# nv-tlabs/LION

Hardware: AMD Instinct MI355X
Metric: shapes/sec @1000-step DDIM, Bx2048pts (higher is better)
Workload: dtype f32 (operands of the 3x3x3 voxel convolutions and of the long 1x1 convolutions cut into fp16 hi/lo pairs on the 16-bi...

## Files before the change

include/lion_hip.h:

```cpp
#ifndef LION_HIP_H_
#define LION_HIP_H_

#include <stddef.h>
#include <stdint.h>

#ifdef __cplusplus
extern "C" {
#endif

typedef void *lionStream_t;

#define LION_OK 0
#define LION_EINVAL (-1)
#define LION_EUNSUPPORTED (-2)
#define LION_EWORKSPACE (-3)

int lion_abi_version(void);

size_t lion_avg_voxelize_workspace_bytes(int B, int C, int N, int r);
int lion_avg_voxelize_forward(const float *feat, const int32_t *coords, int B, int C, int N,
                              int r, float *out, int32_t *ind, int32_t *cnt, void *ws,
                              size_t ws_bytes, lionStream_t stream);

int lion_voxelize_points_forward(const float *feat, const float *coords, int B, int C, int N,
// ... 167 lines not shown
int lion_groupnorm_fold(const float *stats, int B, int C, int T, int G, int voxels, const float *gamma,
                        const float *beta, const float *fac, const float *gbias, int ld_fg, float eps,
                        float *A, float *Bs, float *chmean, lionStream_t stream);
size_t lion_conv3d_split_packed_halfs(int Cout, int Cin);
int lion_conv3d_split_pack_weights(const float *w, int Cout, int Cin, uint16_t *wp, lionStream_t stream);
int lion_conv3d_split_stat_tiles(int r, int Cout);
int lion_conv3d_k3_split_forward(const float *x, const uint16_t *wp, const float *bias, int B, int Cin, int Cout,
                                 int r, const float *pro_a, const float *pro_b, const float *pro_bias,
                                 const float *tconst, float *y, float *stats, int32_t *occ, lionStream_t stream);
int lion_conv3d_k3_half_forward(const float *x, const uint16_t *wp, const float *bias, int B, int Cin, int Cout,
                                int r, const float *pro_a, const float *pro_b, const float *pro_bias,
                                const float *tconst, float *y, float *stats, int32_t *occ, lionStream_t stream);
size_t lion_skinny_packed_floats(int Cout, int Cin);
int lion_skinny_pack_weights(const float *w, int Cout, int Cin, float *wp, lionStream_t stream);
int lion_skinny_splits(int Cin, int Cout);
int lion_skinny_gemm(const float *pin, int ks_in, const float *bias_in, int act_in, const float *addT,
                     const float *wp, int nb, int Cin, int Cout, float *pout, lionStream_t stream);
int lion_skinny_finish(const float *A, int ks_a, const float *bias_a, const float *Bp, int ks_b, const float *resid,
                       int nb, int C, int mode, float *y, lionStream_t stream);
int lion_skinny_gemm_se_finish(const float *pin, int ks_in, const float *bias_in, int act_in, const float *wp, int nb, int Cin,
                               int Cout, const float *A, int ks_a, const float *bias_a, const float *resid, float *y,
                               lionStream_t stream);
int lion_internal_skinny_gemm_plain(const float *pin, int ks_in, const float *bias_in, int act_in, const float *addT,
                                    const float *wp, int nb, int Cin, int Cout, float *pout, lionStream_t stream);
int lion_internal_skinny_gemm_se_finish_plain(const float *pin, int ks_in, const float *bias_in, int act_in, const float *wp,
                                              int nb, int Cin, int Cout, const float *A, int ks_a, const float *bias_a,
                                              const float *resid, float *y, lionStream_t stream);
int lion_to_channel_major(const float *a, int lda, int Ca, float *oa, const float *b, int ldb, int Cb, float *ob, int B,
                          lionStream_t stream);
int lion_from_channel_major(const float *x, int B, int C, float *y, lionStream_t stream);
int lion_groupnorm_fold_se(const float *stats, int B, int C, int T, int G, int voxels, const float *gamma,
                           const float *beta, const float *fac, const float *gbias, int ld_fg, float eps, const float *w1,
                           const float *w2, int H, float *A, float *Bs, lionStream_t stream);
int lion_se_gate(const float *chmean, const float *w1, const float *w2, int B, int C, int H, float *A,
                 float *Bs, lionStream_t stream);
int lion_trilinear_devoxelize_affine_forward(const float *coords, const float *feat, const float *scale,
                                             const float *shift, int B, int C, int N, int r, float *out,
                                             lionStream_t stream);
size_t lion_devoxelize_plan_bytes(int B, int N, int r);
int lion_trilinear_devoxelize_plan(const float *coords, int B, int N, int r, void *plan, size_t plan_bytes,
                                   lionStream_t stream);
int lion_trilinear_devoxelize_planned_forward(const void *plan, size_t plan_bytes, const float *coords, const float *feat,
                                              const float *scale, const float *shift, int B, int C, int N, int r,
                                              float *out, lionStream_t stream);

int lion_row_stats(const float *x, int rows, int L, float *stats, lionStream_t stream);
size_t lion_pwconv_packed_floats(int Cout, int Cin);
int lion_pwconv_pack_weights(const float *w, int Cout, int Cin, float *wp, lionStream_t stream);
int lion_pwconv_stat_tiles(int Cout, int Cin, int L);
int lion_pwconv_forward(const float *x, const float *wp, const float *bias, int B, int Cin, int Cout, int L,
                        const float *pro_a, const float *pro_b, float *y, float *stats, lionStream_t stream);
int lion_pwconv_forward_max(const float *x, const float *wp, const float *bias, int B, int Cin, int Cout, int L,
                            const float *pro_a, const float *pro_b, const float *out_a, const float *out_b,
                            float *stats, float *ymax, lionStream_t stream);
size_t lion_pwconv_split_packed_halfs(int Cout, int Cin);
int lion_pwconv_split_pack_weights(const float *w, int Cout, int Cin, uint16_t *wp, lionStream_t stream);
int lion_pwconv_split_pack_weights_t(const float *w, int Cout, int Cin, const uint16_t *wp, uint16_t *wpt, lionStream_t stream);
int lion_pwconv_split_stat_tiles(int Cout, int Cin, int L);
int lion_pwconv_split_forward(const float *x, const uint16_t *wp, const float *bias, int B, int Cin, int Cout, int L,
                              const float *pro_a, const float *pro_b, float *y, float *stats, lionStream_t stream);
int lion_pwconv_grouped_forward(const float *coords, const float *centers, const float *feat, const int32_t *idx,
                                const float *wp, const float *bias, int B, int C, int N, int M, int U, int Cout, float *y,
                                float *stats, lionStream_t stream);
int lion_pwconv_split_grouped_forward(const float *coords, const float *centers, const float *feat, const int32_t *idx,
                                      const uint16_t *wp, const float *bias, int B, int C, int N, int M, int U, int Cout,
                                      float *y, float *stats, lionStream_t stream);
int lion_internal_pwconv_walk(const float *x, const float *wp, const float *bias, int B, int Cin, int Cout, int L,
                              const float *pro_a, const float *pro_b, const float *out_a, const float *out_b,
                              const float *coords, const float *centers, const float *feat, const int32_t *idx, int N, int U,
                              float *y, float *stats, int max_wg, int lds_weights, lionStream_t stream);
int lion_linear_attention_core(const float *qkv, int B, int H, int D, int N, float *out, lionStream_t stream);
int lion_internal_linear_attention_path(int N, int aligned);
int lion_internal_linear_attention_core_plain(const float *qkv, int B, int H, int D, int N, float *out, lionStream_t stream);
int lion_linear_attention_core_backward(const float *qkv, const float *gout, int B, int H, int D, int N, float *gqkv,
                                        lionStream_t stream);
int lion_linear_forward(const float *x, const float *wp, const float *bias, int B, int K, int O, int act, float slope,
                        float *y, lionStream_t stream);
int lion_affine_swish(const float *x, const float *A, const float *Bs, int rows, int L, float *y,
                      lionStream_t stream);
int lion_affine_swish_max(const float *x, const float *A, const float *Bs, int rows, int M, int U,
                          float *y, lionStream_t stream);
int lion_timestep_embedding(const float *t, const float *row, float scale, int B, int half, int D, float *emb,
                            lionStream_t stream);
int lion_affine_swish_add(const float *x, const float *A, const float *Bs, const float *addend, int rows, int L, float *y,
                          lionStream_t stream);

size_t lion_scatter_csr_workspace_bytes(int B, int E, int bins);
int lion_scatter_csr(const float *gy, const int32_t *idx, const float *w, int B, int C, int S, int E, int bins, void *ws,
                     size_t ws_bytes, float *gx, lionStream_t stream);

size_t lion_pwconv_wgrad_workspace_bytes(int B, int Cin, int Cout, int L);
int lion_pwconv_wgrad(const float *x, const float *gy, int B, int Cin, int Cout, int L, void *ws, size_t ws_bytes,
                      float *gw, float *gb, lionStream_t stream);

int lion_gn_train_fold(const float *stats, const float *gw, const float *gb, const float *fac, int fac_stride,
                       const float *bias, int bias_stride, int B, int C, int G, int L, float eps, float *A, float *Bs,
                       float *mean, float *rstd, lionStream_t stream);
int lion_row_stats64(const float *x, int rows, int L, double *stats, lionStream_t stream);
int lion_gn_train_fold64(const double *stats, const float *gw, const float *gb, const float *fac, int fac_stride,
                         const float *bias, int bias_stride, int B, int C, int G, int L, float eps, float *A,
                         float *Bs, float *mean, float *rstd, lionStream_t stream);
int lion_gn_train_bwd_fold(const float *S, const float *mean, const float *rstd, const float *gw, const float *gb,
                           const float *fac, int fac_stride, int B, int C, int G, int L, float *Q, float *R, float *dfac,
// ... 74 lines not shown
```

lion_amd/_lib.py:

```python
from __future__ import annotations

import ctypes as C
import os

_HERE = os.path.dirname(os.path.abspath(__file__))
SO_PATH = os.environ.get("LION_HIP_SO") or os.path.join(_HERE, "csrc", "liblion_hip.so")

_vp, _i, _f, _sz = C.c_void_p, C.c_int, C.c_float, C.c_size_t

SIGNATURES = {
    "lion_abi_version": (_i, []),
    "lion_avg_voxelize_workspace_bytes": (_sz, [_i, _i, _i, _i]),
    "lion_avg_voxelize_forward": (_i, [_vp, _vp, _i, _i, _i, _i, _vp, _vp, _vp, _vp, _sz, _vp]),
    "lion_voxelize_points_forward": (_i, [_vp, _vp, _i, _i, _i, _i, _i, _f, _vp, _vp, _vp, _vp,
                                          _vp, _sz, _vp]),
    "lion_voxel_plan_bytes": (_sz, [_i, _i, _i]),
    "lion_voxel_index": (_i, [_vp, _i, _i, _i, _i, _f, _vp, _vp, _vp, _vp, _sz, _vp]),
    "lion_voxel_scatter": (_i, [_vp, _vp, _sz, _i, _i, _i, _i, _vp, _vp]),
    "lion_voxel_scatter_read": (_i, [_vp, _vp, _sz, _i, _i, _i, _i, _vp, _vp, _vp]),
    "lion_avg_voxelize_backward": (_i, [_vp, _vp, _vp, _i, _i, _i, _i, _vp, _vp]),
    "lion_trilinear_devoxelize_forward": (_i, [_vp, _vp, _i, _i, _i, _i, _i, _vp, _vp, _vp, _vp]),
    "lion_trilinear_devoxelize_backward": (_i, [_vp, _vp, _vp, _i, _i, _i, _i, _vp, _vp]),
    "lion_ball_query": (_i, [_vp, _vp, _i, _i, _i, _f, _i, _vp, _vp]),
    "lion_grouping_forward": (_i, [_vp, _vp, _i, _i, _i, _i, _i, _vp, _vp]),
# ... 4 lines not shown
    "lion_gather_features_backward": (_i, [_vp, _vp, _i, _i, _i, _i, _vp, _vp]),
    "lion_three_nn_interpolate_forward": (_i, [_vp, _vp, _vp, _i, _i, _i, _i, _vp, _vp, _vp, _vp]),
    "lion_three_nn_interpolate_backward": (_i, [_vp, _vp, _vp, _i, _i, _i, _i, _vp, _vp]),
    "lion_chamfer_forward": (_i, [_vp, _vp, _i, _i, _i, _vp, _vp, _vp, _vp, _vp]),
    "lion_chamfer_backward": (_i, [_vp, _vp, _vp, _vp, _vp, _vp, _i, _i, _i, _vp, _vp, _vp]),
    "lion_chamfer_loss_reduce": (_i, [_vp, _vp, _i, _i, _i, _f, _f, _vp, _vp]),
    "lion_chamfer_loss_backward": (_i, [_vp, _vp, _vp, _vp, _vp, _i, _i, _i, _f, _f, _vp, _vp, _vp]),
    "lion_emd_workspace_bytes": (_sz, [_i, _i, _i]),
    "lion_emd_approxmatch": (_i, [_vp, _vp, _i, _i, _i, _vp, _vp, _sz, _vp]),
    "lion_emd_cost": (_i, [_vp, _vp, _i, _i, _i, _vp, _vp, _sz, _vp]),
    "lion_emd_matchcost": (_i, [_vp, _vp, _vp, _i, _i, _i, _vp, _vp, _sz, _vp]),
    "lion_emd_matchcost_backward": (_i, [_vp, _vp, _vp, _vp, _i, _i, _i, _vp, _vp, _vp]),
    "lion_conv3d_packed_floats": (_sz, [_i, _i]),
    "lion_conv3d_pack_weights": (_i, [_vp, _i, _i, _vp, _vp]),
    "lion_conv3d_k3_forward": (_i, [_vp, _vp, _vp, _i, _i, _i, _i, _vp, _vp]),
    "lion_conv3d_wgrad_workspace_floats": (_sz, [_i, _i, _i, _i]),
    "lion_conv3d_k3_wgrad": (_i, [_vp, _vp, _i, _i, _i, _i, _vp, _vp, _sz, _vp]),
    "lion_conv3d_k3_wgrad_split": (_i, [_vp, _vp, _i, _i, _i, _i, _vp, _vp, _sz, _vp]),
    "lion_conv3d_wgrad_sparse_workspace_floats": (_sz, [_i, _i, _i, _i]),
    "lion_conv3d_k3_wgrad_split_sparse": (_i, [_vp, _vp, _vp, _i, _i, _i, _i, _vp, _vp, _sz, _vp]),
    "lion_conv3d_stat_tiles": (_i, [_i, _i, _i, _i]),
    "lion_conv3d_k3_fused_forward": (_i, [_vp, _vp, _vp, _i, _i, _i, _i, _vp, _vp, _vp, _vp, _vp, _vp, _vp, _vp]),
    "lion_conv3d_const_response": (_i, [_vp, _vp, _vp, _vp, _vp, _i, _i, _i, _vp, _vp]),
    "lion_conv3d_occupancy_ints": (_sz, [_i, _i, _i]),
    "lion_conv3d_tile_occupancy": (_i, [_vp, _i, _i, _i, _vp, _vp, _vp]),
    "lion_conv3d_tile_occupancy_aware": (_i, [_vp, _i, _i, _i, _vp, _vp, _i, _vp]),
    "lion_conv3d_split_packed_halfs": (_sz, [_i, _i]),
    "lion_conv3d_split_pack_weights": (_i, [_vp, _i, _i, _vp, _vp]),
    "lion_conv3d_split_stat_tiles": (_i, [_i, _i]),
    "lion_conv3d_k3_split_forward": (_i, [_vp, _vp, _vp, _i, _i, _i, _i, _vp, _vp, _vp, _vp, _vp, _vp, _vp, _vp]),
    "lion_conv3d_k3_half_forward": (_i, [_vp, _vp, _vp, _i, _i, _i, _i, _vp, _vp, _vp, _vp, _vp, _vp, _vp, _vp]),
    "lion_groupnorm_fold": (_i, [_vp, _i, _i, _i, _i, _i, _vp, _vp, _vp, _vp, _i, _f, _vp, _vp, _vp, _vp]),
    "lion_groupnorm_fold_se": (_i, [_vp, _i, _i, _i, _i, _i, _vp, _vp, _vp, _vp, _i, _f, _vp, _vp, _i, _vp, _vp, _vp]),
    "lion_skinny_packed_floats": (_sz, [_i, _i]),
    "lion_skinny_pack_weights": (_i, [_vp, _i, _i, _vp, _vp]),
    "lion_skinny_splits": (_i, [_i, _i]),
    "lion_skinny_gemm": (_i, [_vp, _i, _vp, _i, _vp, _vp, _i, _i, _i, _vp, _vp]),
    "lion_skinny_gemm_se_finish": (_i, [_vp, _i, _vp, _i, _vp, _i, _i, _i, _vp, _i, _vp, _vp, _vp, _vp]),
    "lion_internal_skinny_gemm_plain": (_i, [_vp, _i, _vp, _i, _vp, _vp, _i, _i, _i, _vp, _vp]),
    "lion_internal_skinny_gemm_se_finish_plain": (_i, [_vp, _i, _vp, _i, _vp, _i, _i, _i, _vp, _i, _vp, _vp, _vp, _vp]),
    "lion_skinny_finish": (_i, [_vp, _i, _vp, _vp, _i, _vp, _i, _i, _i, _vp, _vp]),
    "lion_to_channel_major": (_i, [_vp, _i, _i, _vp, _vp, _i, _i, _vp, _i, _vp]),
    "lion_from_channel_major": (_i, [_vp, _i, _i, _vp, _vp]),
    "lion_se_gate": (_i, [_vp, _vp, _vp, _i, _i, _i, _vp, _vp, _vp]),
    "lion_trilinear_devoxelize_affine_forward": (_i, [_vp, _vp, _vp, _vp, _i, _i, _i, _i, _vp, _vp]),
    "lion_devoxelize_plan_bytes": (_sz, [_i, _i, _i]),
    "lion_trilinear_devoxelize_plan": (_i, [_vp, _i, _i, _i, _vp, _sz, _vp]),
    "lion_trilinear_devoxelize_planned_forward": (_i, [_vp, _sz, _vp, _vp, _vp, _vp, _i, _i, _i, _i, _vp, _vp]),
    "lion_row_stats": (_i, [_vp, _i, _i, _vp, _vp]),
    "lion_pwconv_packed_floats": (_sz, [_i, _i]),
    "lion_pwconv_pack_weights": (_i, [_vp, _i, _i, _vp, _vp]),
    "lion_pwconv_stat_tiles": (_i, [_i, _i, _i]),
    "lion_pwconv_forward": (_i, [_vp, _vp, _vp, _i, _i, _i, _i, _vp, _vp, _vp, _vp, _vp]),
    "lion_pwconv_forward_max": (_i, [_vp, _vp, _vp, _i, _i, _i, _i, _vp, _vp, _vp, _vp, _vp, _vp, _vp]),
    "lion_pwconv_split_packed_halfs": (_sz, [_i, _i]),
    "lion_pwconv_split_pack_weights": (_i, [_vp, _i, _i, _vp, _vp]),
    "lion_pwconv_split_pack_weights_t": (_i, [_vp, _i, _i, _vp, _vp, _vp]),
    "lion_pwconv_split_stat_tiles": (_i, [_i, _i, _i]),
    "lion_pwconv_split_forward": (_i, [_vp, _vp, _vp, _i, _i, _i, _i, _vp, _vp, _vp, _vp, _vp]),
    "lion_pwconv_grouped_forward": (_i, [_vp, _vp, _vp, _vp, _vp, _vp, _i, _i, _i, _i, _i, _i, _vp, _vp, _vp]),
    "lion_pwconv_split_grouped_forward": (_i, [_vp, _vp, _vp, _vp, _vp, _vp, _i, _i, _i, _i, _i, _i, _vp, _vp, _vp]),
    "lion_internal_pwconv_walk": (_i, [_vp, _vp, _vp, _i, _i, _i, _i, _vp, _vp, _vp, _vp, _vp, _vp, _vp, _vp, _i, _i, _vp, _vp, _i, _i, _vp]),
    "lion_linear_attention_core": (_i, [_vp, _i, _i, _i, _i, _vp, _vp]),
    "lion_internal_linear_attention_path": (_i, [_i, _i]),
    "lion_internal_linear_attention_core_plain": (_i, [_vp, _i, _i, _i, _i, _vp, _vp]),
    "lion_linear_attention_core_backward": (_i, [_vp, _vp, _i, _i, _i, _i, _vp, _vp]),
    "lion_linear_forward": (_i, [_vp, _vp, _vp, _i, _i, _i, _i, _f, _vp, _vp]),
    "lion_affine_swish": (_i, [_vp, _vp, _vp, _i, _i, _vp, _vp]),
    "lion_affine_swish_max": (_i, [_vp, _vp, _vp, _i, _i, _i, _vp, _vp]),
    "lion_timestep_embedding": (_i, [_vp, _vp, _f, _i, _i, _i, _vp, _vp]),
    "lion_affine_swish_add": (_i, [_vp, _vp, _vp, _vp, _i, _i, _vp, _vp]),
    "lion_scatter_csr_workspace_bytes": (_sz, [_i, _i, _i]),
    "lion_scatter_csr": (_i, [_vp, _vp, _vp, _i, _i, _i, _i, _i, _vp, _sz, _vp, _vp]),
    "lion_pwconv_wgrad_workspace_bytes": (_sz, [_i, _i, _i, _i]),
    "lion_pwconv_wgrad": (_i, [_vp, _vp, _i, _i, _i, _i, _vp, _sz, _vp, _vp, _vp]),
    "lion_gn_train_fold": (_i, [_vp, _vp, _vp, _vp, _i, _vp, _i, _i, _i, _i, _i, _f, _vp, _vp, _vp, _vp, _vp]),
    "lion_row_stats64": (_i, [_vp, _i, _i, _vp, _vp]),
    "lion_gn_train_fold64": (_i, [_vp, _vp, _vp, _vp, _i, _vp, _i, _i, _i, _i, _i, _f, _vp, _vp, _vp, _vp, _vp]),
    "lion_gn_train_bwd_fold": (_i, [_vp, _vp, _vp, _vp, _vp, _vp, _i, _i, _i, _i, _i, _vp, _vp, _vp, _vp, _i, _vp, _vp, _vp, _vp, _vp,
                                    _vp, _vp]),
    "lion_gn_train_param_grads": (_i, [_vp, _i, _i, _vp, _vp, _vp, _vp]),
    "lion_adam_chunk": (_i, []),
    "lion_adam_row": (_i, []),
    "lion_adam_step": (_i, [_vp, _vp, _vp, _i, _i, _vp, _f, _f, _f, _f, _f, _vp]),
    "lion_grad_sqnorm_partials": (_i, [_vp, _vp, _vp, _i, _vp, _vp]),
    "lion_grad_clip_coef": (_i, [_vp, _i, _f, _vp, _vp]),
    "lion_adam_step_scaled": (_i, [_vp, _vp, _vp, _i, _i, _vp, _f, _f, _f, _f, _f, _vp, _vp]),
    "lion_se_gate_fwd": (_i, [_vp, _vp, _vp, _i, _i, _i, _i, _vp, _vp, _vp, _vp, _vp]),
    "lion_se_gate_bwd": (_i, [_vp, _vp, _vp, _vp, _vp, _vp, _i, _i, _i, _i, _vp, _vp, _vp, _vp, _vp, _vp]),
    "lion_rows_dot2": (_i, [_vp, _vp, _vp, _i, _i, _i, _vp, _vp]),
    "lion_trilinear_devoxelize_backward_affine": (_i, [_vp, _vp, _vp, _vp, _vp, _vp, _vp, _i, _i, _i, _i, _vp, _vp]),
    "lion_gn_se_gate_fwd": (_i, [_vp, _vp, _vp, _vp, _vp, _i, _i, _i, _i, _vp, _vp, _vp, _vp, _vp, _vp]),
    "lion_gn_se_gate_bwd": (_i, [_vp, _vp, _vp, _vp, _vp, _vp, _vp, _vp, _vp, _i, _i, _i, _i, _vp, _vp, _vp, _vp, _vp, _vp, _vp]),
    "lion_affine_act": (_i, [_vp, _vp, _vp, _i, _i, _i, _vp, _vp]),
    "lion_affine_act_bwd_stats": (_i, [_vp, _vp, _vp, _vp, _i, _i, _i, _vp, _vp]),
# ... 119 lines not shown
```

lion_amd/csrc/conv3d.hip:

```cpp
#include "conv3d_tiles.h"

namespace {

typedef float f32x16 __attribute__((ext_vector_type(16)));
#ifndef LION_CONV_KC
#define LION_CONV_KC 4
#endif
#ifndef LION_CONV_WAVES
#define LION_CONV_WAVES 2
#endif
constexpr int KC = LION_CONV_KC;

__device__ __forceinline__ float pro_act(float v, float pa, float pb) {
  const float t = v * pa + pb;
  return swish_fast(t);
}

template <int TD, int TH, int TW, int COT, int VB, bool PRO, bool STATS>
__global__ __launch_bounds__(256, LION_CONV_WAVES) void conv3d_k3_kernel(const float *__restrict__ x,
                                                                const float *__restrict__ wp,
                                                                const float *__restrict__ bias,
                                                                float *__restrict__ y, int Cin,
                                                                int Cout, int r,
                                                                const float *__restrict__ pro_a,
// ... 381 lines not shown
      if (m == 0) {
        if (aware == 2) {
          need = 0;
        } else {
          const int td = t / nth, th = t % nth;
          for (int dd = max(td - 1, 0); dd <= min(td + 1, r / TD - 1); ++dd)
            for (int hh = max(th - 1, 0); hh <= min(th + 1, nth - 1); ++hh) need |= flag[1][dd * nth + hh] != 0;
        }
      }
      fl[t] = f | (need << 8) | ((m == 1 && flag[0][t] != 0) ? (1 << 9) : 0);
      list[f ? before : occupied + (t - before)] = t;
      if (b == 0 && t == 0) { occ[2 * total] = 0; occ[2 * total + 1] = 0; occ[2 * total + 2] = aware; }
    }
  }
}

__global__ __launch_bounds__(256) void conv_tconst_kernel(const float *__restrict__ wsum, const float *__restrict__ bias2,
                                                          const float *__restrict__ bias1, const float *__restrict__ pro_a,
                                                          const float *__restrict__ pro_b, int Cin, int Cout,
                                                          float *__restrict__ tconst) {
  __shared__ float sc[256];
  const int cfg = blockIdx.x, b = blockIdx.y, tid = threadIdx.x;
  for (int c = tid; c < Cin; c += 256)
    sc[c] = pro_act(bias1 ? bias1[c] : 0.f, pro_a[(size_t)b * Cin + c], pro_b[(size_t)b * Cin + c]);
  __syncthreads();
  for (int co = tid; co < Cout; co += 256) {
    double acc = bias2 ? (double)bias2[co] : 0.0;
    const float *w = wsum + (size_t)cfg * Cin * Cout + co;
    for (int c = 0; c < Cin; ++c) acc += (double)w[(size_t)c * Cout] * (double)sc[c];
    tconst[((size_t)b * 27 + cfg) * Cout + co] = (float)acc;
  }
}

__global__ void conv3d_pack_kernel(const float *__restrict__ w, int Cout, int Cin, int Cin_pad,
                                   float *__restrict__ wp) {
  const int i = blockIdx.x * blockDim.x + threadIdx.x;
  const int total = Cin_pad * 27 * Cout;
  if (i >= total) return;
  const int co = i % Cout, t = (i / Cout) % 27, ci = i / (Cout * 27);
  wp[i] = ci < Cin ? w[((size_t)co * Cin + ci) * 27 + t] : 0.f;
}

template <int COT, int TD, int TH, int TW>
static int launch_conv(IntC<TD>, IntC<TH>, IntC<TW>, const float *x, const float *wp, const float *bias, float *y, int B,
                       int Cin, int Cout, int r, const float *pa, const float *pb, const float *pbias, const float *tconst,
                       float *stats, int32_t *occ, hipStream_t st) {
  constexpr int VB = TD * TH * TW / 128;
  const int tiles = conv_tile_count(r, VB);
  dim3 grid;
  if (int e = conv_grid(occ != nullptr, B, tiles, Cout / COT, 2, &grid)) return e;
  constexpr int NT = 256, HALO = (TD + 2) * (TH + 2) * (TW + 2);
  constexpr int SWS = ((KC * 27 * COT + 255) / 256) * 256 + 256;
  static_assert(KC * HALO >= 27 * COT, "the response table must fit the input tile buffer");
  const size_t LDS = (size_t)(((KC * HALO + 3) & ~3) + 2 * SWS + COT + (pa ? 3 * ((Cin + 63) & ~63) : 0) +
                              (NT / 64) * COT * 2) * 4;
  return lion_with_flags(pa != nullptr, stats != nullptr, [&](auto PRO, auto ST) {
    return lion_launch<conv3d_k3_kernel<TD, TH, TW, COT, VB, decltype(PRO)::value, decltype(ST)::value>>(
        grid, NT, LDS, st, x, wp, bias, y, Cin, Cout, r, pa, pb, pbias, tconst, stats, occ, B, tiles);
  });
}

struct ConvPlan { int vb, cot, tiles; };
constexpr ConvPlan conv_plan(int r, int Cout, int B, bool sparse) {
  const int t4 = conv_tile_count(r, 4), t2 = conv_tile_count(r, 2);
  if (!sparse && Cout % 64 == 0 && r >= 16 && (long)t4 * (Cout / 64) * B >= 512) return {4, 64, t4};
  if (Cout % 64 == 0 && (long)t2 * (Cout / 64) * B >= 512) return {2, 64, t2};
// ... 48 lines not shown
                               const float *pro_b, int B, int Cin, int Cout, float *tconst, lionStream_t stream) {
  if (!wsum || !pro_a || !pro_b || !tconst || B <= 0 || Cin <= 0 || Cout <= 0) return LION_EINVAL;
  if (Cin > 256) return LION_EUNSUPPORTED;
  return lion_launch<conv_tconst_kernel>(dim3(27, B), 256, 0, static_cast<hipStream_t>(stream), wsum, bias2, bias1,
                                         pro_a, pro_b, Cin, Cout, tconst);
}

size_t lion_conv3d_occupancy_ints(int r, int Cout, int B) {
  if (r != 16 && r != 32) return 0;
  return (size_t)2 * B * conv_plan(r, Cout, B, true).tiles + 4;
}

int lion_conv3d_tile_occupancy(const int32_t *cnt, int B, int r, int Cout, int32_t *occ_m1, int32_t *occ_m2,
                               lionStream_t stream) {
  return lion_conv3d_tile_occupancy_aware(cnt, B, r, Cout, occ_m1, occ_m2, 0, stream);
}

int lion_conv3d_tile_occupancy_aware(const int32_t *cnt, int B, int r, int Cout, int32_t *occ_m1, int32_t *occ_m2,
                                     int consumer_aware, lionStream_t stream) {
  if (!cnt || (!occ_m1 && !occ_m2) || B <= 0 || Cout <= 0) return LION_EINVAL;
  if (r != 16 && r != 32) return LION_EUNSUPPORTED;
  const ConvPlan p = conv_plan(r, Cout, B, true);
  if (!p.vb || p.tiles > 256 || (((uintptr_t)cnt) & 15) != 0) return LION_EUNSUPPORTED;
  const ConvTileDims t = conv_tile_dims(r, p.vb);
  return lion_launch<conv_tile_occ_kernel>(B, 1024, 0, static_cast<hipStream_t>(stream), cnt, r, t.td, t.th, occ_m1, occ_m2,
                                           consumer_aware == 2 ? 2 : consumer_aware ? 1 : 0);
}

int lion_conv3d_stat_tiles(int r, int Cout, int B, int sparse) {
  if (r != 8 && r != 16 && r != 32) return 0;
  return conv_plan(r, Cout, B, sparse != 0).tiles;
}

int lion_groupnorm_fold_se(const float *stats, int B, int C, int T, int G, int voxels, const float *gamma,
                           const float *beta, const float *fac, const float *gbias, int ld_fg, float eps, const float *w1,
                           const float *w2, int H, float *A, float *Bs, lionStream_t stream) {
  if (!stats || !gamma || !beta || !fac || !gbias || !w1 || !w2 || !A || !Bs) return LION_EINVAL;
  if (B <= 0 || C <= 0 || T <= 0 || G <= 0 || C % G != 0 || ld_fg < C || H <= 0) return LION_EINVAL;
  if (C > 256 || C < 4 || H > 128) return LION_EUNSUPPORTED;
  return lion_launch<gn_fold_se_kernel>(B, 256, 0, static_cast<hipStream_t>(stream), stats, C, T, G, (float)voxels,
                                        gamma, beta, fac, gbias, ld_fg, eps, w1, w2, H, A, Bs);
}

int lion_groupnorm_fold(const float *stats, int B, int C, int T, int G, int voxels, const float *gamma,
                        const float *beta, const float *fac, const float *gbias, int ld_fg, float eps,
                        float *A, float *Bs, float *chmean, lionStream_t stream) {
  if (!stats || !gamma || !beta || !fac || !gbias || !A || !Bs || !chmean) return LION_EINVAL;
  if (B <= 0 || C <= 0 || T <= 0 || G <= 0 || C % G != 0 || C / G > 64 || ld_fg < C) return LION_EINVAL;
  return lion_launch<gn_fold_kernel>(dim3(G, B), 256, 0, static_cast<hipStream_t>(stream), stats, C, T, G,
                                     (float)voxels, gamma, beta, fac, gbias, ld_fg, eps, A, Bs, chmean);
}

}
```

lion_amd/csrc/pwconv.hip:

```cpp
#include "common.h"
#include <algorithm>

namespace {

typedef float f32x16 __attribute__((ext_vector_type(16)));

__device__ __forceinline__ PwGather pw_gather() { return PwGather{}; }
__device__ __forceinline__ PwGather pw_gather(const PwGather &g) { return g; }
template <int CB, int VB, bool PRO, bool STATS, bool WLDS, int OUT = 0, typename... G>
__global__ __launch_bounds__(256, 2) void pwconv_kernel(const float *__restrict__ x, const float *__restrict__ wp,
                                                        const float *__restrict__ bias, float *__restrict__ y,
                                                        int Cin, int Cout, int CoutY, int L,
                                                        const float *__restrict__ pro_a,
                                                        const float *__restrict__ pro_b, float *__restrict__ stats,
                                                        const float *__restrict__ out_a = nullptr,
                                                        const float *__restrict__ out_b = nullptr, G... gather) {
  constexpr bool GRP = sizeof...(G) > 0;
  static_assert(!(GRP && (PRO || OUT)), "the gathered operand is a first layer: no prologue, stored output");
  [[maybe_unused]] const PwGather g = pw_gather(gather...);
  constexpr int COUT = CB * 32;
  extern __shared__ __attribute__((aligned(16))) float smem[];
  const int ksteps = (Cin + 1) >> 1;
  float *sw = smem;
  float *spa = sw + (WLDS ? 2 * ksteps * COUT : 0);
// ... 351 lines not shown
      v = (s0 + u < s_hi && k < Cin && cok) ? v : 0.f;
      acc[0] = __builtin_amdgcn_mfma_f32_32x32x2f32(av[u][0], v, acc[0], 0, 0, 0);
      acc[1] = __builtin_amdgcn_mfma_f32_32x32x2f32(av[u][1], v, acc[1], 0, 0, 0);
    }
  }
#pragma unroll
  for (int cb = 0; cb < 2; ++cb)
#pragma unroll
    for (int i = 0; i < 16; ++i) part[wave][cb][((i & 3) + 8 * (i >> 2) + 4 * kh) * 32 + cl] = acc[cb][i];
  __syncthreads();
  const int c = tid & 31, colo = blockIdx.x * 32 + c;
  const bool ok = colo < L;
  float *yb = y + ((size_t)b * CoutY + co0) * L;
#pragma unroll
  for (int j = 0; j < 8; ++j) {
    const int row = (tid >> 5) + 8 * j, cb = row >> 5, e = (row & 31) * 32 + c;
    float o = ((part[0][cb][e] + part[1][cb][e]) + part[2][cb][e]) + part[3][cb][e];
    const bool rok = co0 + row < CoutY;
    o += brow[j];
    if (ok && rok) yb[(size_t)row * L + colo] = o;
    if (STATS) {
      float s1 = ok ? o : 0.f, s2 = s1 * s1;
      s1 = row16_sum_rn(s1); s2 = row16_sum_rn(s2);
      s1 = row_pair_sum_odd_rows(s1); s2 = row_pair_sum_odd_rows(s2);
      if (c == 16 && rok) {
        float *so = stats + (((size_t)b * CoutY + co0 + row) * gridDim.x + blockIdx.x) * 2;
        so[0] = s1;
        so[1] = s2;
      }
    }
  }
}

__global__ __launch_bounds__(256) void linear_rows_kernel(const float *__restrict__ x, const float *__restrict__ wp,
                                                          const float *__restrict__ bias, int Bn, int K, int O,
                                                          int Opad, int act, float slope, float *__restrict__ y) {
  __shared__ float part[4][1024];
  const int tid = threadIdx.x, lane = tid & 63, wave = tid >> 6, cl = lane & 31, kh = lane >> 5;
  const int o0 = blockIdx.x * 32, b0 = blockIdx.y * 32;
  const int ksteps = (K + 1) >> 1, per = (ksteps + 3) >> 2;
  const int s_lo = min(ksteps, wave * per), s_hi = min(ksteps, s_lo + per);
  const int brow = min(b0 + cl, Bn - 1);
  f32x16 acc;
#pragma unroll
  for (int i = 0; i < 16; ++i) acc[i] = 0.f;
  for (int s = s_lo; s < s_hi; ++s) {
    const int k = 2 * s + kh, kc = min(k, K - 1);
    const float a = wp[(size_t)k * Opad + o0 + cl];
    const float v = (k < K && b0 + cl < Bn) ? x[(size_t)brow * K + kc] : 0.f;
    acc = __builtin_amdgcn_mfma_f32_32x32x2f32(a, v, acc, 0, 0, 0);
  }
#pragma unroll
  for (int i = 0; i < 16; ++i) part[wave][((i & 3) + 8 * (i >> 2) + 4 * kh) * 32 + cl] = acc[i];
  __syncthreads();
#pragma unroll
  for (int e = tid; e < 1024; e += 256) {
    const int o = o0 + (e >> 5), b = b0 + (e & 31);
    if (o < O && b < Bn) {
      float v = ((part[0][e] + part[1][e]) + part[2][e]) + part[3][e];
      if (bias) v += bias[o];
      if (act == 1) v = v > 0.f ? v : 0.f;
      else if (act == 2) v = v > 0.f ? v : v * slope;
      y[(size_t)b * O + o] = v;
    }
  }
}
// ... 53 lines not shown
  PwGather g = {};
  PwSched o = {};
};
template <PwForm FORM, typename F> static int pw_with_form(const PwCall &c, F f) {
  if constexpr (FORM == PW_GATHER) {
    return lion_with_flags(c.stats != nullptr, [&](auto ST) { return f(BoolC<false>{}, ST, IntC<0>{}, c.g); });
  } else if constexpr (FORM == PW_MAX) {
    return lion_with_flags(c.pa != nullptr, c.oa != nullptr, [&](auto PRO, auto SECOND) {
      constexpr bool second = decltype(SECOND)::value;
      return f(PRO, BoolC<!second>{}, IntC<second ? 2 : 1>{});
    });
  } else {
    return lion_with_flags(c.pa != nullptr, c.stats != nullptr, [&](auto PRO, auto ST) { return f(PRO, ST, IntC<0>{}); });
  }
}

template <PwForm FORM, int CB, int VB> static int launch_pw(const PwCall &c, IntC<CB>, IntC<VB>) {
  const int gy = pw_pad(c.Cout) / (CB * 32), tiles = lion_cdiv(c.L, 4 * VB * 32);
  const dim3 grid(pw_grid_x(tiles, gy, c.B, c.o), gy, c.B);
  const bool many = (long)tiles * c.B >= 2048;
  if (FORM == PW_MAX && c.o.wlds < 0 && !many) return LION_EUNSUPPORTED;
  const bool wlds = c.o.wlds < 0 ? many : c.o.wlds != 0;
  const size_t lds = pw_lds(CB, c.Cin, c.pa != nullptr, wlds);
  return pw_with_form<FORM>(c, [&](auto PRO, auto ST, auto OUT, auto... gather) {
    return lion_with_flags(wlds, [&](auto WLDS) {
      return lion_launch<pwconv_kernel<CB, VB, decltype(PRO)::value, decltype(ST)::value, decltype(WLDS)::value,
                                       decltype(OUT)::value, decltype(gather)...>>(
          grid, 256, lds, c.st, c.x, c.wp, c.bias, c.y, c.Cin, pw_stride(c.Cout), c.Cout, c.L, c.pa, c.pb, c.stats, c.oa, c.ob,
          gather...);
    });
  });
}

template <PwForm FORM> static int launch_pw_small(const PwCall &c) {
  const dim3 grid(lion_cdiv(c.L, 32), pw_stride(c.Cout) / 64, c.B);
  const size_t lds = c.pa ? (size_t)2 * c.Cin * 4 : 0;
  if (lds > 64 * 1024) return LION_EUNSUPPORTED;
  return pw_with_form<FORM>(c, [&](auto PRO, auto ST, auto, auto... gather) {
    return lion_launch<pwconv_small_kernel<decltype(PRO)::value, decltype(ST)::value, decltype(gather)...>>(
        grid, 256, lds, c.st, c.x, c.wp, c.bias, c.y, c.Cin, pw_stride(c.Cout), c.Cout, c.L, c.pa, c.pb, c.stats, gather...);
  });
}

}

extern "C" {

int lion_pwconv_forward_max(const float *x, const float *wp, const float *bias, int B, int Cin, int Cout, int L,
                            const float *pro_a, const float *pro_b, const float *out_a, const float *out_b, float *stats,
                            float *ymax, lionStream_t stream) {
  if (!x || !wp || B <= 0 || Cin <= 0 || Cout <= 0 || L <= 0) return LION_EINVAL;
  if ((pro_a == nullptr) != (pro_b == nullptr) || (out_a == nullptr) != (out_b == nullptr)) return LION_EINVAL;
  if (out_a ? !ymax : !stats) return LION_EINVAL;
  if (L % 32 != 0 || L <= PW_SMALL_L || L >= PW_MAX_L) return LION_EUNSUPPORTED;
  const PwPlan p = pw_plan(Cout, Cin);
  if (!p.cb) return LION_EUNSUPPORTED;
  const PwCall c{x, wp, bias, ymax, stats, B, Cin, Cout, L, static_cast<hipStream_t>(stream), pro_a, pro_b, out_a, out_b};
  return pw_with_plan(p, [&](auto CB, auto VB) { return launch_pw<PW_MAX>(c, CB, VB); });
}

size_t lion_pwconv_packed_floats(int Cout, int Cin) { return (size_t)((Cin + 1) / 2 * 2) * pw_stride(Cout); }

int lion_pwconv_pack_weights(const float *w, int Cout, int Cin, float *wp, lionStream_t stream) {
  if (!w || !wp || Cout <= 0 || Cin <= 0) return LION_EINVAL;
  const int Cin_pad = (Cin + 1) / 2 * 2, Cout_pad = pw_stride(Cout);
  return lion_launch<pwconv_pack_kernel>(lion_cdiv(Cin_pad * Cout_pad, 256), 256, 0, static_cast<hipStream_t>(stream),
                                         w, Cout, Cout_pad, Cin, Cin_pad, wp);
}

int lion_pwconv_stat_tiles(int Cout, int Cin, int L) {
  if (L > 0 && L <= PW_SMALL_L && Cout > 0 && Cin > 0) return lion_cdiv(L, 32);
  const PwPlan p = pw_plan(Cout, Cin);
  return (p.cb && L > 0 && L < PW_MAX_L) ? lion_cdiv(L, 4 * p.vb * 32) : 0;
// ... 18 lines not shown
  if ((long)M * U >= (1L << 31) || (long)C * N >= (1L << 31)) return LION_EUNSUPPORTED;
  const int Cin = 3 + C, L = M * U;
  PwCall c{nullptr, wp, bias, y, stats, B, Cin, Cout, L, static_cast<hipStream_t>(stream)};
  c.g = PwGather{coords, centers, C > 0 ? feat : nullptr, idx, C, N, U};
  if (L <= PW_SMALL_L) return launch_pw_small<PW_GATHER>(c);
  const PwPlan p = pw_plan(Cout, Cin);
  if (!p.cb || L >= PW_MAX_L || N >= PW_MAX_L) return LION_EUNSUPPORTED;
  return pw_with_plan(p, [&](auto CB, auto VB) { return launch_pw<PW_GATHER>(c, CB, VB); });
}

int lion_internal_pwconv_walk(const float *x, const float *wp, const float *bias, int B, int Cin, int Cout, int L,
                              const float *pro_a, const float *pro_b, const float *out_a, const float *out_b,
                              const float *coords, const float *centers, const float *feat, const int32_t *idx, int N, int U,
                              float *y, float *stats, int max_wg, int lds_weights, lionStream_t stream) {
  if (!wp || B <= 0 || Cin <= 0 || Cout <= 0 || L <= 0) return LION_EINVAL;
  if ((pro_a == nullptr) != (pro_b == nullptr) || (out_a == nullptr) != (out_b == nullptr)) return LION_EINVAL;
  const bool grouped = idx != nullptr, maxform = out_a || !y;
  if (out_a ? !y : (!y && !stats)) return LION_EINVAL;
  if (grouped ? (!coords || !centers || N <= 0 || U <= 0 || L % U != 0 || Cin < 3 || (Cin > 3 && !feat) || pro_a || maxform) : !x)
    return LION_EINVAL;
  if ((maxform && L % 32 != 0) || L >= PW_MAX_L || (grouped && N >= PW_MAX_L)) return LION_EUNSUPPORTED;
  const PwPlan p = pw_plan(Cout, Cin);
  if (!p.cb) return LION_EUNSUPPORTED;
  const PwCall c{grouped ? nullptr : x, wp, bias, y, stats, B, Cin, Cout, L, static_cast<hipStream_t>(stream),
                 pro_a, pro_b, out_a, out_b, PwGather{coords, centers, Cin > 3 ? feat : nullptr, idx, Cin - 3, N, U},
                 PwSched{max_wg, lds_weights}};
  return pw_with_plan(p, [&](auto CB, auto VB) {
    if (grouped) return launch_pw<PW_GATHER>(c, CB, VB);
    if (maxform) return launch_pw<PW_MAX>(c, CB, VB);
    return launch_pw<PW_STORE>(c, CB, VB);
  });
}

int lion_linear_forward(const float *x, const float *wp, const float *bias, int B, int K, int O, int act, float slope,
                        float *y, lionStream_t stream) {
  if (!x || !wp || !y || B <= 0 || K <= 0 || O <= 0 || act < 0 || act > 2) return LION_EINVAL;
  const int Opad = pw_stride(O);
  return lion_launch<linear_rows_kernel>(dim3(pw_pad(O) / 32, lion_cdiv(B, 32)), 256, 0,
                                         static_cast<hipStream_t>(stream), x, wp, bias, B, K, O, Opad, act, slope, y);
}

}
```

Baseline: 5.808.

## Issue loads ahead of compute in small pwconv and GroupNorm-SE fold kernels

Adds a small-L pointwise-conv kernel variant that loads all weight and activation operands for a wave's K-slice into registers before the MFMA loop, with double-buffered prefetch when Cin is large. It also adds a GroupNorm+SE fold kernel that preloads the SE weights and per-channel parameters into registers ahead of the stats reduction and parallelizes the first SE matvec across waves. Both aim to hide global load latency in latency-bound small launches, at the cost of higher register pressure. The previous kernels stay reachable through internal plain entry points.

Result: faster. 5.901 (median of 6 runs) (+1.6%).

```diff
diff --git a/include/lion_hip.h b/include/lion_hip.h
--- a/include/lion_hip.h
+++ b/include/lion_hip.h
@@ -223,6 +223,9 @@
 int lion_groupnorm_fold_se(const float *stats, int B, int C, int T, int G, int voxels, const float *gamma,
                            const float *beta, const float *fac, const float *gbias, int ld_fg, float eps, const float *w1,
                            const float *w2, int H, float *A, float *Bs, lionStream_t stream);
+int lion_internal_groupnorm_fold_se_plain(const float *stats, int B, int C, int T, int G, int voxels, const float *gamma,
+                                          const float *beta, const float *fac, const float *gbias, int ld_fg, float eps,
+                                          const float *w1, const float *w2, int H, float *A, float *Bs, lionStream_t stream);
 int lion_se_gate(const float *chmean, const float *w1, const float *w2, int B, int C, int H, float *A,
                  float *Bs, lionStream_t stream);
 int lion_trilinear_devoxelize_affine_forward(const float *coords, const float *feat, const float *scale,
@@ -260,6 +263,10 @@
                               const float *pro_a, const float *pro_b, const float *out_a, const float *out_b,
                               const float *coords, const float *centers, const float *feat, const int32_t *idx, int N, int U,
                               float *y, float *stats, int max_wg, int lds_weights, lionStream_t stream);
+int lion_internal_pwconv_small_plain(const float *x, const float *wp, const float *bias, int B, int Cin, int Cout, int L,
+                                     const float *pro_a, const float *pro_b, const float *coords, const float *centers,
+                                     const float *feat, const int32_t *idx, int N, int U, float *y, float *stats,
+                                     lionStream_t stream);
 int lion_linear_attention_core(const float *qkv, int B, int H, int D, int N, float *out, lionStream_t stream);
 int lion_internal_linear_attention_path(int N, int aligned);
 int lion_internal_linear_attention_core_plain(const float *qkv, int B, int H, int D, int N, float *out, lionStream_t stream);
diff --git a/lion_amd/_lib.py b/lion_amd/_lib.py
--- a/lion_amd/_lib.py
+++ b/lion_amd/_lib.py
@@ -60,6 +60,7 @@
     "lion_conv3d_k3_half_forward": (_i, [_vp, _vp, _vp, _i, _i, _i, _i, _vp, _vp, _vp, _vp, _vp, _vp, _vp, _vp]),
     "lion_groupnorm_fold": (_i, [_vp, _i, _i, _i, _i, _i, _vp, _vp, _vp, _vp, _i, _f, _vp, _vp, _vp, _vp]),
     "lion_groupnorm_fold_se": (_i, [_vp, _i, _i, _i, _i, _i, _vp, _vp, _vp, _vp, _i, _f, _vp, _vp, _i, _vp, _vp, _vp]),
+    "lion_internal_groupnorm_fold_se_plain": (_i, [_vp, _i, _i, _i, _i, _i, _vp, _vp, _vp, _vp, _i, _f, _vp, _vp, _i, _vp, _vp, _vp]),
     "lion_skinny_packed_floats": (_sz, [_i, _i]),
     "lion_skinny_pack_weights": (_i, [_vp, _i, _i, _vp, _vp]),
     "lion_skinny_splits": (_i, [_i, _i]),
@@ -89,6 +90,7 @@
     "lion_pwconv_grouped_forward": (_i, [_vp, _vp, _vp, _vp, _vp, _vp, _i, _i, _i, _i, _i, _i, _vp, _vp, _vp]),
     "lion_pwconv_split_grouped_forward": (_i, [_vp, _vp, _vp, _vp, _vp, _vp, _i, _i, _i, _i, _i, _i, _vp, _vp, _vp]),
     "lion_internal_pwconv_walk": (_i, [_vp, _vp, _vp, _i, _i, _i, _i, _vp, _vp, _vp, _vp, _vp, _vp, _vp, _vp, _i, _i, _vp, _vp, _i, _i, _vp]),
+    "lion_internal_pwconv_small_plain": (_i, [_vp, _vp, _vp, _i, _i, _i, _i, _vp, _vp, _vp, _vp, _vp, _vp, _i, _i, _vp, _vp, _vp]),
     "lion_linear_attention_core": (_i, [_vp, _i, _i, _i, _i, _vp, _vp]),
     "lion_internal_linear_attention_path": (_i, [_i, _i]),
     "lion_internal_linear_attention_core_plain": (_i, [_vp, _i, _i, _i, _i, _vp, _vp]),
diff --git a/lion_amd/csrc/conv3d.hip b/lion_amd/csrc/conv3d.hip
--- a/lion_amd/csrc/conv3d.hip
+++ b/lion_amd/csrc/conv3d.hip
@@ -437,6 +437,86 @@
   }
 }
 
+template <int HV, int CC>
+__global__ __launch_bounds__(256) void gn_fold_se_ahead_kernel(const float *__restrict__ stats, int C, int T, int G, float count,
+                                                               const float *__restrict__ gamma, const float *__restrict__ beta,
+                                                               const float *__restrict__ fac, const float *__restrict__ gbias,
+                                                               int ld_fg, float eps, const float *__restrict__ w1,
+                                                               const float *__restrict__ w2, float *__restrict__ A,
+                                                               float *__restrict__ Bs) {
+  constexpr int H = 4 * HV;
+  __shared__ double cs[256][2];
+  __shared__ float sA[256], sB[256], sm[256], sh[128];
+  const int b = blockIdx.x, tid = threadIdx.x, lane = tid & 63, wave = tid >> 6, cpg = C / G;
+  const int tc = min(tid, C - 1);
+  const float p_f = fac[(size_t)b * ld_fg + tc], p_gb = gbias[(size_t)b * ld_fg + tc], p_gam = gamma[tc], p_bet = beta[tc];
+  float w1r[HV][CC];
+  float4 w2r[HV];
+#pragma unroll
+  for (int jj = 0; jj < HV; ++jj)
+#pragma unroll
+    for (int q = 0; q < CC; ++q) w1r[jj][q] = w1[(size_t)(wave + 4 * jj) * C + min(lane + 64 * q, C - 1)];
+#pragma unroll
+  for (int j = 0; j < HV; ++j) w2r[j] = reinterpret_cast<const float4 *>(w2 + (size_t)tc * H)[j];
+  int cp2 = 1;
+  while (cp2 < C) cp2 <<= 1;
+  const int LPC = 256 / cp2, ch = tid / LPC, sub = tid % LPC;
+  double s1 = 0.0, s2 = 0.0;
+  if (ch < C) {
+    const float2 *p = reinterpret_cast<const float2 *>(stats + (((size_t)b * C + ch) * T) * 2);
+    for (int t0 = sub; t0 < T; t0 += 8 * LPC) {
+      float2 v[8];
+#pragma unroll
+      for (int u = 0; u < 8; ++u) v[u] = p[min(t0 + u * LPC, T - 1)];
+#pragma unroll
+      for (int u = 0; u < 8; ++u)
+        if (t0 + u * LPC < T) { s1 += (double)v[u].x; s2 += (double)v[u].y; }
+    }
+  }
+  for (int m = 1; m < LPC; m <<= 1) { s1 += __shfl_xor(s1, m, 64); s2 += __shfl_xor(s2, m, 64); }
+  if (ch < C && sub == 0) { cs[ch][0] = s1; cs[ch][1] = s2; }
+  __syncthreads();
+  if (tid < C) {
+    const int g0 = (tid / cpg) * cpg;
+    double g1 = 0.0, g2 = 0.0;
+    for (int k = 0; k < cpg; ++k) { g1 += cs[g0 + k][0]; g2 += cs[g0 + k][1]; }
+    const double n = (double)count * cpg, mean = g1 / n;
+    double var = g2 / n - mean * mean;
+    var = var > 0.0 ? var : 0.0;
+    const float rstd = (float)(1.0 / sqrt(var + (double)eps));
+    const float a0 = rstd * p_gam;
+    const float a = a0 * p_f, bb = (p_bet - (float)mean * a0) * p_f + p_gb;
+    sA[tid] = a;
+    sB[tid] = bb;
+    sm[tid] = a * (float)(cs[tid][0] / count) + bb;
+  }
+  __syncthreads();
+#pragma unroll
+  for (int jj = 0; jj < HV; ++jj) {
+    float acc = 0.f;
+#pragma unroll
+    for (int q = 0; q < CC; ++q)
+      if (lane + 64 * q < C) acc += w1r[jj][q] * sm[lane + 64 * q];
+#pragma unroll
+    for (int m = 32; m >= 1; m >>= 1) acc += __shfl_xor(acc, m, 64);
+    if (lane == 0) sh[wave + 4 * jj] = acc > 0.f ? acc : 0.f;
+  }
+  __syncthreads();
+  if (tid < C) {
+    float acc = 0.f;
+#pragma unroll
+    for (int j = 0; j < HV; ++j) {
+      acc += w2r[j].x * sh[4 * j];
+      acc += w2r[j].y * sh[4 * j + 1];
+      acc += w2r[j].z * sh[4 * j + 2];
+      acc += w2r[j].w * sh[4 * j + 3];
+    }
+    const float g = 1.0f / (1.0f + expf(-acc));
+    A[(size_t)b * C + tid] = sA[tid] * g;
+    Bs[(size_t)b * C + tid] = sB[tid] * g;
+  }
+}
+
 __global__ void conv3d_pack_kernel(const float *__restrict__ w, int Cout, int Cin, int Cin_pad,
                                    float *__restrict__ wp) {
   const int i = blockIdx.x * blockDim.x + threadIdx.x;
@@ -551,12 +631,37 @@
   return conv_plan(r, Cout, B, sparse != 0).tiles;
 }
 
+static int gn_fold_se_args(const float *stats, int B, int C, int T, int G, const float *gamma, const float *beta,
+                           const float *fac, const float *gbias, int ld_fg, const float *w1, const float *w2, int H,
+                           float *A, float *Bs) {
+  if (!stats || !gamma || !beta || !fac || !gbias || !w1 || !w2 || !A || !Bs) return LION_EINVAL;
+  if (B <= 0 || C <= 0 || T <= 0 || G <= 0 || C % G != 0 || ld_fg < C || H <= 0) return LION_EINVAL;
+  if (C > 256 || C < 4 || H > 128) return LION_EUNSUPPORTED;
+  return 0;
+}
+
 int lion_groupnorm_fold_se(const float *stats, int B, int C, int T, int G, int voxels, const float *gamma,
                            const float *beta, const float *fac, const float *gbias, int ld_fg, float eps, const float *w1,
                            const float *w2, int H, float *A, float *Bs, lionStream_t stream) {
-  if (!stats || !gamma || !beta || !fac || !gbias || !w1 || !w2 || !A || !Bs) return LION_EINVAL;
-  if (B <= 0 || C <= 0 || T <= 0 || G <= 0 || C % G != 0 || ld_fg < C || H <= 0) return LION_EINVAL;
-  if (C > 256 || C < 4 || H > 128) return LION_EUNSUPPORTED;
+  if (int e = gn_fold_se_args(stats, B, C, T, G, gamma, beta, fac, gbias, ld_fg, w1, w2, H, A, Bs)) return e;
+  hipStream_t st = static_cast<hipStream_t>(stream);
+  if (H % 4 != 0 || H > 32 || (H & (H - 1)) != 0 || (((uintptr_t)w2) & 15) != 0)
+    return lion_launch<gn_fold_se_kernel>(B, 256, 0, st, stats, C, T, G, (float)voxels, gamma, beta, fac, gbias, ld_fg, eps, w1, w2,
+                                          H, A, Bs);
+  auto go = [&](auto HV, auto CC) {
+    return lion_launch<gn_fold_se_ahead_kernel<decltype(HV)::value, decltype(CC)::value>>(
+        B, 256, 0, st, stats, C, T, G, (float)voxels, gamma, beta, fac, gbias, ld_fg, eps, w1, w2, A, Bs);
+  };
+  auto rows = [&](auto CC) {
+    return H == 4 ? go(IntC<1>{}, CC) : H == 8 ? go(IntC<2>{}, CC) : H == 16 ? go(IntC<4>{}, CC) : go(IntC<8>{}, CC);
+  };
+  return C <= 64 ? rows(IntC<1>{}) : C <= 128 ? rows(IntC<2>{}) : rows(IntC<4>{});
+}
+
+int lion_internal_groupnorm_fold_se_plain(const float *stats, int B, int C, int T, int G, int voxels, const float *gamma,
+                                          const float *beta, const float *fac, const float *gbias, int ld_fg, float eps,
+                                          const float *w1, const float *w2, int H, float *A, float *Bs, lionStream_t stream) {
+  if (int e = gn_fold_se_args(stats, B, C, T, G, gamma, beta, fac, gbias, ld_fg, w1, w2, H, A, Bs)) return e;
   return lion_launch<gn_fold_se_kernel>(B, 256, 0, static_cast<hipStream_t>(stream), stats, C, T, G, (float)voxels,
                                         gamma, beta, fac, gbias, ld_fg, eps, w1, w2, H, A, Bs);
 }
diff --git a/lion_amd/csrc/pwconv.hip b/lion_amd/csrc/pwconv.hip
--- a/lion_amd/csrc/pwconv.hip
+++ b/lion_amd/csrc/pwconv.hip
@@ -407,6 +407,134 @@
   }
 }
 
+template <bool PRO, bool STATS, bool MR, typename... G>
+__global__ __launch_bounds__(256) void pwconv_small_ahead_kernel(const float *__restrict__ x, const float *__restrict__ wp,
+                                                                 const float *__restrict__ bias, float *__restrict__ y,
+                                                                 int Cin, int Cout, int CoutY, int L,
+                                                                 const float *__restrict__ pro_a,
+                                                                 const float *__restrict__ pro_b, float *__restrict__ stats,
+                                                                 G... gather) {
+  constexpr bool GRP = sizeof...(G) > 0;
+  static_assert(!(GRP && PRO), "the gathered operand is a first layer: no prologue");
+  [[maybe_unused]] const PwGather g = pw_gather(gather...);
+  __shared__ float part[4][2][1024];
+  extern __shared__ __attribute__((aligned(16))) float smem[];
+  const int tid = threadIdx.x, lane = tid & 63, wave = tid >> 6, cl = lane & 31, kh = lane >> 5;
+  const int b = blockIdx.z, co0 = blockIdx.y * 64, col = blockIdx.x * 32 + cl;
+  const bool cok = col < L;
+  const int colc = cok ? col : L - 1;
+  const int ksteps = (Cin + 1) >> 1, per = (ksteps + 3) >> 2;
+  const int s_lo = min(ksteps, wave * per), s_hi = min(ksteps, s_lo + per);
+  float *spa = smem, *spb = smem + Cin;
+  [[maybe_unused]] float ra = 0.f, rb = 0.f;
+  if (PRO && !MR) {
+    ra = pro_a[(size_t)b * Cin + min(tid, Cin - 1)];
+    rb = pro_b[(size_t)b * Cin + min(tid, Cin - 1)];
+  }
+  const float *xb = x + (size_t)b * Cin * L;
+  int gi = 0;
+  float gc0 = 0.f, gc1 = 0.f;
+  const float *gcb = nullptr, *gfb = nullptr;
+  int gfr = 0;
+  if constexpr (GRP) {
+    const int M = L / g.U, m = colc / g.U;
+    gcb = g.coords + (size_t)b * 3 * g.N;
+    gfb = g.feat ? g.feat + (size_t)b * g.C * g.N : gcb;
+    gfr = g.feat ? g.C - 1 : 0;
+    gc0 = g.centers[((size_t)b * 3 + kh) * M + m];
+    gc1 = g.centers[((size_t)b * 3 + 2) * M + m];
+    gi = min(max(g.idx[(size_t)b * L + colc], 0), g.N - 1);
+  }
+  constexpr int UN = MR ? 16 : 32;
+  auto load = [&](int s0, float (&av)[UN][2], float (&bv)[UN]) __attribute__((always_inline)) {
+#pragma unroll
+    for (int u = 0; u < UN; ++u) {
+      const int k = min(2 * min(s0 + u, ksteps - 1) + kh, 2 * ksteps - 1);
+      av[u][0] = wp[(size_t)k * Cout + co0 + cl];
+      av[u][1] = wp[(size_t)k * Cout + co0 + 32 + cl];
+      if constexpr (GRP) {
+        const int kc = min(k, Cin - 1);
+        const float *row = kc < 3 ? gcb + (size_t)kc * g.N : gfb + (size_t)min(max(kc - 3, 0), gfr) * g.N;
+        bv[u] = row[gi];
+      } else {
+        bv[u] = xb[(size_t)min(k, Cin - 1) * L + colc];
+      }
+    }
+  };
+  f32x16 acc[2];
+#pragma unroll
+  for (int cb = 0; cb < 2; ++cb)
+#pragma unroll
+    for (int i = 0; i < 16; ++i) acc[cb][i] = 0.f;
+  auto mma = [&](int s0, const float (&av)[UN][2], const float (&bv)[UN]) __attribute__((always_inline)) {
+#pragma unroll
+    for (int u = 0; u < UN; ++u) {
+      const int k = 2 * (s0 + u) + kh;
+      float v = bv[u];
+      if (PRO) {
+        const int kc = min(k, Cin - 1);
+        const float t = v * spa[kc] + spb[kc];
+        v = swish_fast(t);
+      }
+      if constexpr (GRP) v = k < 3 ? sub_rn(v, k == 2 ? gc1 : gc0) : v;
+      v = (s0 + u < s_hi && k < Cin && cok) ? v : 0.f;
+      acc[0] = __builtin_amdgcn_mfma_f32_32x32x2f32(av[u][0], v, acc[0], 0, 0, 0);
+      acc[1] = __builtin_amdgcn_mfma_f32_32x32x2f32(av[u][1], v, acc[1], 0, 0, 0);
+    }
+  };
+  float av0[UN][2], bv0[UN];
+  load(s_lo, av0, bv0);
+  float brow[8];
+#pragma unroll
+  for (int j = 0; j < 8; ++j) brow[j] = (bias && co0 + (tid >> 5) + 8 * j < CoutY) ? bias[co0 + (tid >> 5) + 8 * j] : 0.f;
+  if (PRO) {
+    if (MR) {
+      for (int c = tid; c < Cin; c += 256) { spa[c] = pro_a[(size_t)b * Cin + c]; spb[c] = pro_b[(size_t)b * Cin + c]; }
+    } else if (tid < Cin) {
+      spa[tid] = ra;
+      spb[tid] = rb;
+    }
+    __syncthreads();
+  }
+  if constexpr (MR) {
+    float av1[UN][2], bv1[UN];
+    for (int s0 = s_lo; s0 < s_hi; s0 += 2 * UN) {
+      load(s0 + UN, av1, bv1);
+      mma(s0, av0, bv0);
+      load(s0 + 2 * UN, av0, bv0);
+      if (s0 + UN < s_hi) mma(s0 + UN, av1, bv1);
+    }
+  } else {
+    if (s_lo < s_hi) mma(s_lo, av0, bv0);
+  }
+#pragma unroll
+  for (int cb = 0; cb < 2; ++cb)
+#pragma unroll
+    for (int i = 0; i < 16; ++i) part[wave][cb][((i & 3) + 8 * (i >> 2) + 4 * kh) * 32 + cl] = acc[cb][i];
+  __syncthreads();
+  const int c = tid & 31, colo = blockIdx.x * 32 + c;
+  const bool ok = colo < L;
+  float *yb = y + ((size_t)b * CoutY + co0) * L;
+#pragma unroll
+  for (int j = 0; j < 8; ++j) {
+    const int row = (tid >> 5) + 8 * j, cb = row >> 5, e = (row & 31) * 32 + c;
+    float o = ((part[0][cb][e] + part[1][cb][e]) + part[2][cb][e]) + part[3][cb][e];
+    const bool rok = co0 + row < CoutY;
+    o += brow[j];
+    if (ok && rok) yb[(size_t)row * L + colo] = o;
+    if (STATS) {
+      float s1 = ok ? o : 0.f, s2 = s1 * s1;
+      s1 = row16_sum_rn(s1); s2 = row16_sum_rn(s2);
+      s1 = row_pair_sum_odd_rows(s1); s2 = row_pair_sum_odd_rows(s2);
+      if (c == 16 && rok) {
+        float *so = stats + (((size_t)b * CoutY + co0 + row) * gridDim.x + blockIdx.x) * 2;
+        so[0] = s1;
+        so[1] = s2;
+      }
+    }
+  }
+}
+
 __global__ __launch_bounds__(256) void linear_rows_kernel(const float *__restrict__ x, const float *__restrict__ wp,
                                                           const float *__restrict__ bias, int Bn, int K, int O,
                                                           int Opad, int act, float slope, float *__restrict__ y) {
@@ -526,13 +654,19 @@
   });
 }
 
-template <PwForm FORM> static int launch_pw_small(const PwCall &c) {
+template <PwForm FORM> static int launch_pw_small(const PwCall &c, bool plain = false) {
   const dim3 grid(lion_cdiv(c.L, 32), pw_stride(c.Cout) / 64, c.B);
   const size_t lds = c.pa ? (size_t)2 * c.Cin * 4 : 0;
   if (lds > 64 * 1024) return LION_EUNSUPPORTED;
   return pw_with_form<FORM>(c, [&](auto PRO, auto ST, auto, auto... gather) {
-    return lion_launch<pwconv_small_kernel<decltype(PRO)::value, decltype(ST)::value, decltype(gather)...>>(
-        grid, 256, lds, c.st, c.x, c.wp, c.bias, c.y, c.Cin, pw_stride(c.Cout), c.Cout, c.L, c.pa, c.pb, c.stats, gather...);
+    if (plain)
+      return lion_launch<pwconv_small_kernel<decltype(PRO)::value, decltype(ST)::value, decltype(gather)...>>(
+          grid, 256, lds, c.st, c.x, c.wp, c.bias, c.y, c.Cin, pw_stride(c.Cout), c.Cout, c.L, c.pa, c.pb, c.stats, gather...);
+    return lion_with_flags(c.Cin > 256, [&](auto MR) {
+      return lion_launch<pwconv_small_ahead_kernel<decltype(PRO)::value, decltype(ST)::value, decltype(MR)::value,
+                                                   decltype(gather)...>>(
+          grid, 256, lds, c.st, c.x, c.wp, c.bias, c.y, c.Cin, pw_stride(c.Cout), c.Cout, c.L, c.pa, c.pb, c.stats, gather...);
+    });
   });
 }
 
@@ -617,6 +751,22 @@
   });
 }
 
+int lion_internal_pwconv_small_plain(const float *x, const float *wp, const float *bias, int B, int Cin, int Cout, int L,
+                                     const float *pro_a, const float *pro_b, const float *coords, const float *centers,
+                                     const float *feat, const int32_t *idx, int N, int U, float *y, float *stats,
+                                     lionStream_t stream) {
+  if (!wp || !y || B <= 0 || Cin <= 0 || Cout <= 0 || L <= 0) return LION_EINVAL;
+  if ((pro_a == nullptr) != (pro_b == nullptr)) return LION_EINVAL;
+  const bool grouped = idx != nullptr;
+  if (grouped ? (!coords || !centers || N <= 0 || U <= 0 || L % U != 0 || Cin < 3 || (Cin > 3 && !feat) || pro_a) : !x)
+    return LION_EINVAL;
+  if (L > PW_SMALL_L) return LION_EUNSUPPORTED;
+  PwCall c{grouped ? nullptr : x, wp, bias, y, stats, B, Cin, Cout, L, static_cast<hipStream_t>(stream), pro_a, pro_b};
+  if (!grouped) return launch_pw_small<PW_STORE>(c, true);
+  c.g = PwGather{coords, centers, Cin > 3 ? feat : nullptr, idx, Cin - 3, N, U};
+  return launch_pw_small<PW_GATHER>(c, true);
+}
+
 int lion_linear_forward(const float *x, const float *wp, const float *bias, int B, int K, int O, int act, float slope,
                         float *y, lionStream_t stream) {
   if (!x || !wp || !y || B <= 0 || K <= 0 || O <= 0 || act < 0 || act > 2) return LION_EINVAL;
```
